# slp-rl/slamkit

Hardware: AMD Instinct MI355X
Metric: train tokens/sec (whole node), Slam-358M ctx=1024 (higher is better)
Workload: dtype bf16; 1 GPU; configs[1]: Slam-358M (Qwen2.5-0.5B body, vocab 502, rope_theta 1e4), ctx=1024, synthetic unit-token stream, random-init weights; full optimizer step (AdamW on bf16 parameters with bf16 moments); model=Slam-358M, global_batch=8, micro_batch=8, seq_len=1024, grad_accum=1, parallelism=dp1, optimizer_state_dtype=bfloat16

## Files before the change

### slamkit_amd/csrc/attention.hip

```cpp
#include <type_traits>

#include "common.h"
#include "kernels.h"

namespace {

constexpr int IMG = 64 * 128;
constexpr float NEG_BIG = -1.0e30f;
constexpr float M_INIT = -1.0e29f;
constexpr int NCH_MAX = 4;
constexpr float LN2 = 0.69314718055994530942f;

struct AttnArgs {
  const bf16_t* qkv;
  bf16_t* o;
  const bf16_t* d_o;
  bf16_t* dqkv;
  float* lse2;
  float* ndsum;
  float* nlse;
  float* dkv_part;
  const int* seg_start;
  const int* seg_end;
  const float* rope_cs;
  const float* rope_sn;
  const int* perm;
  int M, nH, nKV, ldq, nch, prio;
  float scale;
};

typedef __attribute__((address_space(3))) const char* lds_cptr_t;
typedef __attribute__((ext_vector_type(4))) unsigned u32x4_t;
typedef __attribute__((address_space(3))) const u32x4_t* lds_u4ptr_t;
SLAM_DEVICE lds_cptr_t lds_p(uint32_t a) { return (lds_cptr_t)(uintptr_t)a; }

SLAM_DEVICE int uni_f(int k) { return ((k & 3) << 1) ^ ((k >> 2) * 5); }

struct TileOff {
  uint32_t v[2];
  int ld, tid;
  SLAM_DEVICE void init(int ld_, int tid_) {
    ld = ld_; tid = tid_;
#pragma unroll
    for (int i = 0; i < 2; ++i) v[i] = off(i, 63);
  }
  SLAM_DEVICE uint32_t off(int i, int maxrow) const {
    int P = i * 256 + tid;
    int row = P >> 3, slot = P & 7;
    int c = slot ^ uni_f((row >> 1) & 7);
    row = row < maxrow ? row : maxrow;
    return (uint32_t)(((size_t)row * ld + c * 8) * sizeof(bf16_t));
  }
};
template <bool FULL>
SLAM_DEVICE void dma_tile64(const bf16_t* tb, const TileOff& to, int maxrow, uint32_t dst) {
#pragma unroll
  for (int i = 0; i < 2; ++i) glds16_m0(tb, FULL ? to.v[i] : to.off(i, maxrow), dst + (uint32_t)(i * 4096));
}

struct FragOff {
  uint32_t d[2], t[4];
  SLAM_DEVICE void init(int l15, int g) {
    const int fk = uni_f(l15 >> 1);
#pragma unroll
    for (int ds = 0; ds < 2; ++ds) d[ds] = (uint32_t)(l15 * 128 + (((g + 4 * ds) ^ fk) << 4));
    const int x = ((l15 & 3) >> 1) ^ uni_f(2 * g + (l15 >> 3));
#pragma unroll
    for (int fd = 0; fd < 4; ++fd)
      t[fd] = (uint32_t)((4 * g + (l15 >> 2)) * 128 + (((2 * fd) ^ x) << 4) + (l15 & 1) * 8);
  }
};
struct TileAddr {
  uint32_t d[2], t[4];
  SLAM_DEVICE void set(const FragOff& fo, uint32_t stage_base) {
#pragma unroll
    for (int i = 0; i < 2; ++i) { d[i] = stage_base + fo.d[i]; asm volatile("" : "+v"(d[i])); }
#pragma unroll
    for (int i = 0; i < 4; ++i) { t[i] = stage_base + fo.t[i]; asm volatile("" : "+v"(t[i])); }
  }
  SLAM_DEVICE uint4 D(int img, int f, int ds) const {
    const u32x4_t v = *(lds_u4ptr_t)(lds_p(d[ds]) + (img + f * 2048));
    return make_uint4(v[0], v[1], v[2], v[3]);
  }
  SLAM_DEVICE uint4 T(int img, int fd, int t2) const {
    lds_cptr_t q = lds_p(t[fd]) + (img + t2 * 4096);
    typedef __attribute__((address_space(3))) s16x4_t* trp_t;
    s16x4_t lo = __builtin_amdgcn_ds_read_tr16_b64_v4i16((trp_t)q);
    s16x4_t hi = __builtin_amdgcn_ds_read_tr16_b64_v4i16((trp_t)(q + 2048));
    uint2 a = __builtin_bit_cast(uint2, lo), b = __builtin_bit_cast(uint2, hi);
    return make_uint4(a.x, a.y, b.x, b.y);
  }
};

SLAM_DEVICE uint4 pack_pair(const f32x4_t& a, const f32x4_t& b) {
  return make_uint4(pack_bf16x2(a[0], a[1]), pack_bf16x2(a[2], a[3]), pack_bf16x2(b[0], b[1]),
                    pack_bf16x2(b[2], b[3]));
}
SLAM_DEVICE void wait_all_loads_visible() { __builtin_amdgcn_s_waitcnt(0x0F70); }

struct BlockItem { int slot, h, kvh; bool valid; };
SLAM_DEVICE BlockItem block_item(int b, int ntile, int nH, int nKV) {
  const int G = nH / nKV;
  const int seq = b >> 3;
  const int cid = (seq / G) * 8 + (b & 7);
  BlockItem it;
  it.valid = cid < ntile * nKV;
  it.kvh = cid % nKV;
  it.slot = cid / nKV;
  it.h = it.kvh * G + seq % G;
  return it;
}
SLAM_DEVICE void set_rank_prio(int rank, int total) {
  const int q = (4 * rank) / (total > 0 ? total : 1);
  if (q <= 0) __builtin_amdgcn_s_setprio(3);
  else if (q == 1) __builtin_amdgcn_s_setprio(2);
  else if (q == 2) __builtin_amdgcn_s_setprio(1);
}
inline int item_grid(int ntile, int nH, int nKV) { return ((ntile * nKV + 7) / 8) * 8 * (nH / nKV); }

template <int ND>
struct FwdCfg {
  static constexpr int NST = ND == 1 ? 3 : 2;
  static constexpr int STAGE = 2 * ND * IMG;
  static constexpr int OCC = ND == 1 ? 3 : 2;
};
template <int ND>
__global__ __launch_bounds__(256, FwdCfg<ND>::OCC) void attn_fwd_kernel(AttnArgs p) {
  constexpr int NST = FwdCfg<ND>::NST, STG = FwdCfg<ND>::STAGE, D = 64 * ND;
  extern __shared__ __attribute__((aligned(16))) char smem[];
  const int tid = threadIdx.x, lane = tid & 63, wave = tid >> 6;
  const int l15 = lane & 15, g = lane >> 4;
  const int M = p.M, ld = p.ldq;
// ... 148 lines not shown
    for (int j = 0; j < 2; ++j) {
      float ps = 0.f;
#pragma unroll
      for (int f = 0; f < 4; ++f)
#pragma unroll
        for (int r = 0; r < 4; ++r) {
          const float e = fast_exp2(st[f][j][r]);
          st[f][j][r] = e;
          ps += e;
        }
      lsum[j] += ps;
      pb[0][j] = pack_pair(st[0][j], st[1][j]);
      pb[1][j] = pack_pair(st[2][j], st[3][j]);
    }
    __builtin_amdgcn_sched_barrier(0);
    uint4 vf1[4 * ND];
#pragma unroll
    for (int fd = 0; fd < 4 * ND; ++fd) vf1[fd] = ta.T((ND + (fd >> 2)) * IMG, fd & 3, 1);
#pragma unroll
    for (int fd = 0; fd < 4 * ND; ++fd)
#pragma unroll
      for (int j = 0; j < 2; ++j) ot[fd][j] = mfma16(vf0[fd], pb[0][j], ot[fd][j]);
#pragma unroll
    for (int fd = 0; fd < 4 * ND; ++fd)
#pragma unroll
      for (int j = 0; j < 2; ++j) ot[fd][j] = mfma16(vf1[fd], pb[1][j], ot[fd][j]);
  }
#pragma unroll
  for (int j = 0; j < 2; ++j) {
    float l = lsum[j];
    l += __shfl_xor(l, 16, 64);
    l += __shfl_xor(l, 32, 64);
    const int q = qrow[j];
    if (q < M) {
      const float inv = 1.f / l;
#pragma unroll
      for (int fd = 0; fd < 4 * ND; ++fd) {
        uint2 o;
        o.x = pack_bf16x2(ot[fd][j][0] * inv, ot[fd][j][1] * inv);
        o.y = pack_bf16x2(ot[fd][j][2] * inv, ot[fd][j][3] * inv);
        *reinterpret_cast<uint2*>(p.o + (size_t)q * (p.nH * D) + h * D + fd * 16 + g * 4) = o;
      }
      if (g == 0 && p.lse2) p.lse2[(size_t)h * M + q] = log2f(l) - negm[j][0];
    }
  }
}

template <int ND, int JQ>
struct DqCfg {
  static constexpr int NST = ND == 1 ? 3 : 2;
  static constexpr int STAGE = 2 * ND * IMG;
  static constexpr int OCC = ND == 1 ? (JQ == 1 ? 3 : 2) : 2;
};
template <int ND, int JQ>
__global__ __launch_bounds__(256, (DqCfg<ND, JQ>::OCC)) void attn_bwd_dq_kernel(AttnArgs p) {
  constexpr int D = 64 * ND, STG = DqCfg<ND, JQ>::STAGE, NST = DqCfg<ND, JQ>::NST, QT = 64 * JQ, WR = 16 * JQ;
  extern __shared__ __attribute__((aligned(16))) char smem[];
  const int tid = threadIdx.x, lane = tid & 63, wave = tid >> 6;
  const int l15 = lane & 15, g = lane >> 4;
  const int M = p.M, ld = p.ldq;
  const BlockItem bi = block_item(blockIdx.x, (M + QT - 1) / QT, p.nH, p.nKV);
  if (!bi.valid) return;
  const int h = bi.h, kvh = bi.kvh;
  const int q0 = (p.perm ? p.perm[bi.slot] : bi.slot) * QT;
  if (p.prio && p.perm) set_rank_prio(bi.slot, (M + QT - 1) / QT);
  const int wv = __builtin_amdgcn_readfirstlane(wave);
  const int qw0 = q0 + wv * WR;
  const bf16_t* Qb = p.qkv + h * D;
  const bf16_t* Kb = p.qkv + (p.nH + kvh) * D;
  const bf16_t* Vb = p.qkv + (p.nH + p.nKV + kvh) * D;
  const float c2 = p.scale * 1.44269504088896340736f;
  const uint32_t lds0 = lds_addr(smem);

  const int kt_begin = p.seg_start[q0 < M ? q0 : M - 1] / 64;
  const int kt_end = (min(q0 + QT - 1, M - 1)) / 64;
  const int n = kt_end - kt_begin + 1;
  TileOff off;
  off.init(ld, tid);
  FragOff fo;
  fo.init(l15, g);
  const size_t tstep = (size_t)64 * ld;
  const bf16_t* kp = Kb + (size_t)kt_begin * tstep;
  const bf16_t* vp = Vb + (size_t)kt_begin * tstep;
  int irow = kt_begin * 64;
  const uint32_t wdst = lds0 + (uint32_t)wv * 1024u;
  auto issue = [&](int stage) __attribute__((always_inline)) {
    const uint32_t st = wdst + (uint32_t)(stage * STG);
    if (irow + 64 <= M) {
#pragma unroll
      for (int dh = 0; dh < ND; ++dh) {
        dma_tile64<true>(kp + dh * 64, off, 63, st + dh * IMG);
        dma_tile64<true>(vp + dh * 64, off, 63, st + (ND + dh) * IMG);
      }
    } else {
      const int mr = M - 1 - irow;
#pragma unroll
      for (int dh = 0; dh < ND; ++dh) {
        dma_tile64<false>(kp + dh * 64, off, mr, st + dh * IMG);
        dma_tile64<false>(vp + dh * 64, off, mr, st + (ND + dh) * IMG);
      }
    }
    kp += tstep; vp += tstep; irow += 64;
  };
#pragma unroll
  for (int s = 0; s < NST - 1; ++s)
    if (s < n) issue(s);

  int qrow[JQ], segs[JQ];
  float lse[JQ], nds[JQ];
  uint4 qf[JQ][2 * ND], dof[JQ][2 * ND];
#pragma unroll
  for (int j = 0; j < JQ; ++j) {
    const int q = qw0 + j * 16 + l15;
    const int qc = q < M ? q : M - 1;
    qrow[j] = q;
    segs[j] = p.seg_start[qc];
    lse[j] = -p.lse2[(size_t)h * M + qc];
    float dsm = 0.f;
#pragma unroll
    for (int ds = 0; ds < 2 * ND; ++ds) {
      qf[j][ds] = *reinterpret_cast<const uint4*>(Qb + (size_t)qc * ld + g * 8 + 32 * ds);
      dof[j][ds] = *reinterpret_cast<const uint4*>(p.d_o + (size_t)qc * p.nH * D + h * D + g * 8 + 32 * ds);
      uint4 of = *reinterpret_cast<const uint4*>(p.o + (size_t)qc * p.nH * D + h * D + g * 8 + 32 * ds);
      float x[8], y[8];
      unpack_bf16x8(dof[j][ds], x);
      unpack_bf16x8(of, y);
#pragma unroll
      for (int e = 0; e < 8; ++e) dsm += x[e] * y[e];
    }
    dsm += __shfl_xor(dsm, 16, 64);
    dsm += __shfl_xor(dsm, 32, 64);
    nds[j] = -dsm;
    if (g == 0 && q < M) {
      p.ndsum[(size_t)h * M + q] = -dsm;
      p.nlse[(size_t)h * M + q] = lse[j];
    }
  }
  const int segmax_w = p.seg_start[min(qw0 + WR - 1, M - 1)];
  f32x4_t dq[JQ][4 * ND];
#pragma unroll
  for (int j = 0; j < JQ; ++j)
#pragma unroll
    for (int fd = 0; fd < 4 * ND; ++fd) dq[j][fd] = (f32x4_t){0.f, 0.f, 0.f, 0.f};
  wait_all_loads_visible();

  int stage = 0, istage = (NST - 1) % NST;
  for (int t = 0; t < n; ++t) {
    if (NST >= 3 && t + 1 < n) wait_vmcnt<4 * ND>();
    else wait_vmcnt<0>();
    __syncthreads();
    if (t + NST - 1 < n) issue(istage);
    istage = istage + 1 == NST ? 0 : istage + 1;
    const uint32_t sb = lds0 + (uint32_t)(stage * STG);
    stage = stage + 1 == NST ? 0 : stage + 1;
    const int key0 = (kt_begin + t) * 64;
    if (key0 > qw0 + WR - 1) continue;
    TileAddr ta;
    ta.set(fo, sb);
    f32x4_t st[4][JQ], dp[4][JQ];
#pragma unroll
    for (int f = 0; f < 4; ++f)
#pragma unroll
      for (int j = 0; j < JQ; ++j) {
        st[f][j] = (f32x4_t){lse[j], lse[j], lse[j], lse[j]};
        dp[f][j] = (f32x4_t){nds[j], nds[j], nds[j], nds[j]};
      }
#pragma unroll
    for (int ds = 0; ds < 2 * ND; ++ds)
#pragma unroll
      for (int f = 0; f < 4; ++f) {
        const uint4 kf = ta.D((ds >> 1) * IMG, f, ds & 1);
        const uint4 vf = ta.D((ND + (ds >> 1)) * IMG, f, ds & 1);
#pragma unroll
        for (int j = 0; j < JQ; ++j) {
          st[f][j] = mfma16(kf, qf[j][ds], st[f][j]);
          dp[f][j] = mfma16(vf, dof[j][ds], dp[f][j]);
        }
      }
    uint4 dsb[2][JQ];
    auto soft = [&](auto mk) __attribute__((always_inline)) {
      constexpr bool MASK = decltype(mk)::value;
#pragma unroll
      for (int j = 0; j < JQ; ++j) {
        int hi = 0, lo = 0;
        if constexpr (MASK) {
          hi = (qrow[j] < M ? qrow[j] : -(1 << 30)) - key0 - 4 * g;
          lo = segs[j] - key0 - 4 * g;
        }
#pragma unroll
        for (int f = 0; f < 4; ++f)
#pragma unroll
          for (int r = 0; r < 4; ++r) {
            float pe = fast_exp2(st[f][j][r]);
            if constexpr (MASK) {
              const bool ok = (f * 16 + r <= hi) & (f * 16 + r >= lo);
              pe = ok ? pe : 0.f;
            }
            st[f][j][r] = pe * dp[f][j][r];
          }
        dsb[0][j] = pack_pair(st[0][j], st[1][j]);
        dsb[1][j] = pack_pair(st[2][j], st[3][j]);
      }
    };
    uint4 kt0[4 * ND];
#pragma unroll
    for (int fd = 0; fd < 4 * ND; ++fd) kt0[fd] = ta.T((fd >> 2) * IMG, fd & 3, 0);
    __builtin_amdgcn_sched_barrier(0);
    if ((key0 + 63 > qw0) || (key0 < segmax_w) || (qw0 + WR - 1 >= M)) soft(std::true_type{});
    else soft(std::false_type{});
    __builtin_amdgcn_sched_barrier(0);
    uint4 kt1[4 * ND];
#pragma unroll
    for (int fd = 0; fd < 4 * ND; ++fd) kt1[fd] = ta.T((fd >> 2) * IMG, fd & 3, 1);
#pragma unroll
    for (int fd = 0; fd < 4 * ND; ++fd)
#pragma unroll
      for (int j = 0; j < JQ; ++j) dq[j][fd] = mfma16(kt0[fd], dsb[0][j], dq[j][fd]);
#pragma unroll
    for (int fd = 0; fd < 4 * ND; ++fd)
#pragma unroll
      for (int j = 0; j < JQ; ++j) dq[j][fd] = mfma16(kt1[fd], dsb[1][j], dq[j][fd]);
  }
#pragma unroll
  for (int j = 0; j < JQ; ++j) {
    const int q = qrow[j];
    if (q < M) {
#pragma unroll
      for (int fd = 0; fd < 4 * ND; ++fd)
#pragma unroll
        for (int r = 0; r < 4; ++r) dq[j][fd][r] *= p.scale;
      if (p.rope_cs) {
#pragma unroll
        for (int fd = 0; fd < 2 * ND; ++fd) {
          const float4 c4 = *reinterpret_cast<const float4*>(p.rope_cs + (size_t)q * (D / 2) + fd * 16 + g * 4);
          const float4 s4 = *reinterpret_cast<const float4*>(p.rope_sn + (size_t)q * (D / 2) + fd * 16 + g * 4);
          const float cc[4] = {c4.x, c4.y, c4.z, c4.w}, ss[4] = {s4.x, s4.y, s4.z, s4.w};
#pragma unroll
          for (int r = 0; r < 4; ++r) {
            float a = dq[j][fd][r], b = dq[j][fd + 2 * ND][r];
            dq[j][fd][r] = a * cc[r] + b * ss[r];
            dq[j][fd + 2 * ND][r] = b * cc[r] - a * ss[r];
          }
        }
      }
#pragma unroll
      for (int fd = 0; fd < 4 * ND; ++fd) {
        uint2 o;
        o.x = pack_bf16x2(dq[j][fd][0], dq[j][fd][1]);
        o.y = pack_bf16x2(dq[j][fd][2], dq[j][fd][3]);
        *reinterpret_cast<uint2*>(p.dqkv + (size_t)q * ld + h * D + fd * 16 + g * 4) = o;
      }
    }
  }
}

template <int ND, int KW>
struct DkvCfg {
  static constexpr int NST = ND == 1 ? 3 : 2;
  static constexpr int STAGE = 2 * ND * IMG + 1024;
  static constexpr int OCC = ND == 1 ? (KW == 1 ? 3 : 2) : 2;
};
struct DkvRange { int qa, nq, nch; };
SLAM_DEVICE DkvRange dkv_range(const int* seg_end, int M, int k0, int KT, int nchmax, int c) {
  const int qt_begin = k0 / 64;
  const int qt_end = (seg_end[min(k0 + KT - 1, M - 1)] - 1) / 64;
  const int n = qt_end - qt_begin + 1;
  const int cs = (n + nchmax - 1) / nchmax;
  DkvRange r;
  r.nch = (n + cs - 1) / cs;
  r.qa = qt_begin + c * cs;
  r.nq = min(cs, qt_end - r.qa + 1);
  return r;
}
template <int ND, int KW>
__global__ __launch_bounds__(256, (DkvCfg<ND, KW>::OCC)) void attn_bwd_dkv_kernel(AttnArgs p) {
  constexpr int D = 64 * ND, STG = DkvCfg<ND, KW>::STAGE, NST = DkvCfg<ND, KW>::NST, KT = 64 * KW, WK = 16 * KW;
  constexpr int NDMA = 4 * ND + 1;
  extern __shared__ __attribute__((aligned(16))) char smem[];
  const int tid = threadIdx.x, lane = tid & 63, wave = tid >> 6;
  const int l15 = lane & 15, g = lane >> 4;
  const int M = p.M, ld = p.ldq, ldo = p.nH * D;
  const int G = p.nH / p.nKV;
  const int kvh = blockIdx.x % p.nKV;
  const int item = p.perm[blockIdx.x / p.nKV];
  if (item < 0) return;
  if (p.prio) set_rank_prio(blockIdx.x / p.nKV, ((M + KT - 1) / KT) * NCH_MAX);
  const int chunk = item & (NCH_MAX - 1), k0 = (item >> 2) * KT;
  const DkvRange rg = dkv_range(p.seg_end, M, k0, KT, p.nch, chunk);
  const int nq = rg.nq, qa = rg.qa;
  const int n = G * nq;
  const bf16_t* Kb = p.qkv + (p.nH + kvh) * D;
  const bf16_t* Vb = p.qkv + (p.nH + p.nKV + kvh) * D;
  const float c2 = p.scale * 1.44269504088896340736f;
  const uint32_t lds0 = lds_addr(smem);
// ... 207 lines not shown
    }
  }
  if (which == 0 && p.rope_cs) {
    const float4 c4 = *reinterpret_cast<const float4*>(p.rope_cs + (size_t)m * HALF + c * 4);
    const float4 s4 = *reinterpret_cast<const float4*>(p.rope_sn + (size_t)m * HALF + c * 4);
    float4 x = a, y = b;
    a = make_float4(x.x * c4.x + y.x * s4.x, x.y * c4.y + y.y * s4.y, x.z * c4.z + y.z * s4.z, x.w * c4.w + y.w * s4.w);
    b = make_float4(y.x * c4.x - x.x * s4.x, y.y * c4.y - x.y * s4.y, y.z * c4.z - x.z * s4.z, y.w * c4.w - x.w * s4.w);
  }
  uint2 o1, o2;
  o1.x = pack_bf16x2(a.x, a.y); o1.y = pack_bf16x2(a.z, a.w);
  o2.x = pack_bf16x2(b.x, b.y); o2.y = pack_bf16x2(b.z, b.w);
  int col = (p.nH + (which ? p.nKV : 0) + kvh) * D + c * 4;
  *reinterpret_cast<uint2*>(p.dqkv + (size_t)m * p.ldq + col) = o1;
  *reinterpret_cast<uint2*>(p.dqkv + (size_t)m * p.ldq + col + HALF) = o2;
}

__global__ __launch_bounds__(1024) void attn_plan_kernel(const int* __restrict__ seg_s, const int* __restrict__ seg_e, int M, int qt,
                                                        int kt, int nchmax, int* __restrict__ plan) {
  extern __shared__ int wk[];
  const int nf = (M + 127) / 128, nq = (M + qt - 1) / qt, nk = (M + kt - 1) / kt;
  const int total = seg_e ? nf + nq + nk * NCH_MAX : nf;
  for (int t = threadIdx.x; t < total; t += blockDim.x) {
    int w;
    if (t < nf) { int q0 = t * 128; w = min(q0 + 127, M - 1) / 64 - seg_s[q0] / 64 + 1; }
    else if (t < nf + nq) { int q0 = (t - nf) * qt; w = min(q0 + qt - 1, M - 1) / 64 - seg_s[q0] / 64 + 1; }
    else {
      const int j = t - nf - nq, c = j & (NCH_MAX - 1);
      const DkvRange r = dkv_range(seg_e, M, (j >> 2) * kt, kt, nchmax, c);
      w = c < r.nch ? r.nq : -1;
    }
    wk[t] = w;
  }
  __syncthreads();
  for (int t = threadIdx.x; t < total; t += blockDim.x) {
    int base, n;
    if (t < nf) { base = 0; n = nf; }
    else if (t < nf + nq) { base = nf; n = nq; }
    else { base = nf + nq; n = nk * NCH_MAX; }
    const int i = t - base, w = wk[t];
    int rank = 0;
    for (int j = 0; j < n; ++j) {
      const int wj = wk[base + j];
      rank += (wj > w) || (wj == w && j < i);
    }
    plan[base + rank] = (base == nf + nq && w <= 0) ? -1 : i;
  }
}

}

namespace slam {

static AttnTune g_attn_tune = {1, 1, 4, 0};
AttnTune attn_default_tune() { return g_attn_tune; }
void attn_set_default_tune(AttnTune t) { g_attn_tune = t; }
static AttnTune clamp_tune(AttnTune t, int head_dim) {
  t.jq = t.jq == 2 && head_dim == 64 ? 2 : 1;
  t.kw = 1;
  t.nch = t.nch < 1 ? 1 : t.nch > NCH_MAX ? NCH_MAX : t.nch;
  return t;
}

size_t attn_plan_ints(int M) { return (size_t)((M + 127) / 128 + (M + 63) / 64 + NCH_MAX * ((M + 63) / 64)); }
int attn_plan(const int* seg_start, const int* seg_end, int M, int head_dim, AttnTune tune, int* plan, hipStream_t st) {
  tune = clamp_tune(tune, head_dim);
  const int qt = 64 * tune.jq, kt = 64 * tune.kw;
  const int total = (M + 127) / 128 + (M + qt - 1) / qt + NCH_MAX * ((M + kt - 1) / kt);
  if ((size_t)total * sizeof(int) > 48 * 1024) return -1;
  attn_plan_kernel<<<1, 1024, (size_t)total * sizeof(int), st>>>(seg_start, seg_end, M, qt, kt, tune.nch, plan);
  return (int)hipGetLastError();
}

template <typename K>
static int set_lds(K kernel, int bytes) {
  return (int)hipFuncSetAttribute(reinterpret_cast<const void*>(kernel), hipFuncAttributeMaxDynamicSharedMemorySize, bytes);
}

template <int ND>
static int attn_fwd_nd(AttnArgs a, hipStream_t st) {
  static bool done = false;
  constexpr int lds = FwdCfg<ND>::NST * FwdCfg<ND>::STAGE;
  if (!done) { if (int e = set_lds(&attn_fwd_kernel<ND>, lds)) return e; done = true; }
  attn_fwd_kernel<ND><<<item_grid((a.M + 127) / 128, a.nH, a.nKV), 256, lds, st>>>(a);
  return (int)hipGetLastError();
}

template <int ND, int JQ>
static int attn_dq_launch(AttnArgs a, hipStream_t st) {
  static bool done = false;
  constexpr int lds = DqCfg<ND, JQ>::NST * DqCfg<ND, JQ>::STAGE;
  if (!done) { if (int e = set_lds(&attn_bwd_dq_kernel<ND, JQ>, lds)) return e; done = true; }
  attn_bwd_dq_kernel<ND, JQ><<<item_grid((a.M + 64 * JQ - 1) / (64 * JQ), a.nH, a.nKV), 256, lds, st>>>(a);
  return (int)hipGetLastError();
}
template <int ND, int KW>
static int attn_dkv_launch(AttnArgs a, hipStream_t st) {
  static bool done = false;
  constexpr int lds = DkvCfg<ND, KW>::NST * DkvCfg<ND, KW>::STAGE;
  if (!done) { if (int e = set_lds(&attn_bwd_dkv_kernel<ND, KW>, lds)) return e; done = true; }
  const int nk = (a.M + 64 * KW - 1) / (64 * KW);
  attn_bwd_dkv_kernel<ND, KW><<<nk * NCH_MAX * a.nKV, 256, lds, st>>>(a);
  return (int)hipGetLastError();
}

int attn_fwd(const bf16_t* qkv, bf16_t* o, float* lse2, const int* seg_start, const int* plan, AttnTune tune, int M, int nH,
             int nKV, int head_dim, hipStream_t st) {
  if ((head_dim != 64 && head_dim != 128) || nH % nKV) return -1;
  AttnArgs a{};
  a.qkv = qkv; a.o = o; a.lse2 = lse2; a.seg_start = seg_start; a.perm = plan; a.prio = tune.prio;
  a.M = M; a.nH = nH; a.nKV = nKV; a.ldq = (nH + 2 * nKV) * head_dim; a.scale = 1.0f / sqrtf((float)head_dim);
  return head_dim == 64 ? attn_fwd_nd<1>(a, st) : attn_fwd_nd<2>(a, st);
}

size_t attn_bwd_workspace_bytes(int M, int nKV, int head_dim) {
  return (size_t)NCH_MAX * 2 * nKV * M * head_dim * sizeof(float);
}

int attn_bwd(const bf16_t* qkv, const bf16_t* o, const bf16_t* d_o, const float* lse2, float* ndsum, float* nlse,
             bf16_t* dqkv, float* dkv_part, const int* seg_start, const int* seg_end, const int* plan, AttnTune tune,
             const float* rope_cs, const float* rope_sn, int M, int nH, int nKV, int head_dim, hipStream_t st) {
  if ((head_dim != 64 && head_dim != 128) || nH % nKV || !plan) return -1;
  tune = clamp_tune(tune, head_dim);
  AttnArgs a{};
  a.qkv = qkv; a.o = const_cast<bf16_t*>(o); a.d_o = d_o; a.dqkv = dqkv;
  a.lse2 = const_cast<float*>(lse2); a.ndsum = ndsum; a.nlse = nlse; a.dkv_part = dkv_part;
  a.seg_start = seg_start; a.seg_end = seg_end;
  a.rope_cs = rope_cs; a.rope_sn = rope_sn;
  a.M = M; a.nH = nH; a.nKV = nKV; a.ldq = (nH + 2 * nKV) * head_dim; a.scale = 1.0f / sqrtf((float)head_dim);
  a.nch = tune.nch; a.prio = tune.prio;
  const int nf = (M + 127) / 128, qt = 64 * tune.jq, kt = 64 * tune.kw;
  a.perm = plan + nf;
  int e;
  if (head_dim == 128) e = attn_dq_launch<2, 1>(a, st);
  else e = tune.jq == 2 ? attn_dq_launch<1, 2>(a, st) : attn_dq_launch<1, 1>(a, st);
  if (e) return e;
  a.perm = plan + nf + (M + qt - 1) / qt;
  if (head_dim == 128) e = attn_dkv_launch<2, 1>(a, st);
  else e = attn_dkv_launch<1, 1>(a, st);
  if (e) return e;
  const size_t total = (size_t)2 * M * nKV * (head_dim / 8);
  if (head_dim == 128) attn_dkv_reduce_kernel<2><<<(unsigned)((total + 255) / 256), 256, 0, st>>>(a, kt);
  else attn_dkv_reduce_kernel<1><<<(unsigned)((total + 255) / 256), 256, 0, st>>>(a, kt);
  return (int)hipGetLastError();
}

}
```

### slamkit_amd/csrc/engine.hip

```cpp
#include <hip/hip_runtime.h>
#include <math.h>
#include <stdio.h>
#include <dlfcn.h>
#include <string.h>

#include <algorithm>
#include <string>
#include <unordered_map>
#include <utility>
#include <vector>

#if __has_include(<rccl/rccl.h>)
#include <rccl/rccl.h>
#else
typedef struct ncclComm* ncclComm_t;
typedef struct { char internal[128]; } ncclUniqueId;
typedef enum { ncclSuccess = 0 } ncclResult_t;
typedef enum { ncclInt8 = 0, ncclUint8 = 1, ncclInt32 = 2, ncclUint32 = 3, ncclInt64 = 4, ncclUint64 = 5, ncclFloat16 = 6, ncclFloat32 = 7,
               ncclFloat64 = 8, ncclBfloat16 = 9 } ncclDataType_t;
typedef enum { ncclSum = 0 } ncclRedOp_t;
#endif

#include "../../include/slam_engine.h"
#include "kernels.h"
// ... 798 lines not shown
  if (!h->params) return h->fail(SLAM_ESTATE, "bind params first");
  hipStream_t st = (hipStream_t)stream;
  CK(join_optimizer(h, st));
  CK(join_params(h, st));
  h->params_t_dirty = false;
  const auto tr = transpose_group(h, st);
  CK(for_each_param_group(h, 0, tr));
  CK(for_each_param_group(h, h->d.n_layers + 1, tr));
  CK(for_each_layer_tensor(h, 0, h->d.n_layers, tr));
  return SLAM_OK;
}
int slam_bind_params_t(SlamEngine* h, void* params_t_bf16) {
  if (!h) return SLAM_EINVAL;
  const SlamModelDesc& d = h->d;
  if (params_t_bf16 && ((d.hidden & 63) || (d.intermediate & 63) || (h->QKV & 63) || ((d.n_heads * d.head_dim) & 63)))
    return h->fail(SLAM_EINVAL, "transposed weight images need dims that are multiples of 64");
  h->params_t = (bf16_t*)params_t_bf16;
  return SLAM_OK;
}
size_t slam_workspace_bytes(SlamEngine* h, int64_t max_tokens) {
  if (!h || max_tokens <= 0) return 0;
  GemmTuneScope tune_scope(&h->gemm_tune);
  SlamEngine tmp;
  tmp.d = h->d;
  tmp.arch = h->arch;
  tmp.npos = h->npos;
  tmp.QKV = h->QKV;
  tmp.vpad = h->vpad;
  tmp.untied = h->untied;
  tmp.n_params = h->n_params;
  tmp.recompute = h->recompute;
  tmp.dropout_thr16 = h->dropout_thr16;
  return carve(&tmp, nullptr, max_tokens);
}
int slam_bind_workspace(SlamEngine* h, void* ws, size_t bytes, int64_t max_tokens) {
  if (!h || !ws || max_tokens <= 0) return SLAM_EINVAL;
  if (((uintptr_t)ws) & 255) return h->fail(SLAM_EINVAL, "workspace must be 256-byte aligned");
  size_t need = slam_workspace_bytes(h, max_tokens);
  if (bytes < need) return h->fail(SLAM_ENOMEM, "workspace too small");
  carve(h, (char*)ws, max_tokens);
  h->ws = (char*)ws;
  h->ws_bytes = bytes;
  h->max_tokens = max_tokens;
  h->have_fwd = false;
  return SLAM_OK;
}
int slam_set_option(SlamEngine* h, const char* key, int64_t value) {
  if (!key) return SLAM_EINVAL;
  if (!strncmp(key, "gemm_", 5)) {
    const int r = gemm_tune_set(h ? &h->gemm_tune : gemm_default_tune(), key, (long)value);
    if (r > 0) return SLAM_OK;
    return h ? h->fail(SLAM_EINVAL, std::string(r < 0 ? "value out of range for option " : "unknown option ") + key) : SLAM_EINVAL;
  }
  if (!strcmp(key, "attn_jq") || !strcmp(key, "attn_kw") || !strcmp(key, "attn_nch") || !strcmp(key, "attn_prio")) {
    AttnTune t = h ? h->attn_tune : attn_default_tune();
    (key[5] == 'j' ? t.jq : key[5] == 'k' ? t.kw : key[5] == 'n' ? t.nch : t.prio) = (int)value;
    if (h) { h->attn_tune = t; h->have_fwd = false; } else attn_set_default_tune(t);
    return SLAM_OK;
  }
  if (!strcmp(key, "overlap_adamw") && h) { h->overlap_adamw = value != 0; return SLAM_OK; }
  if (!strcmp(key, "adamw_sr") && h) {
    if (value < 0 || value > 1) return h->fail(SLAM_EINVAL, "value out of range for option adamw_sr (0 or 1)");
    h->adamw_sr = (int)value;
    return SLAM_OK;
  }
  if (!strcmp(key, "adamw_sr_seed") && h) { h->adamw_sr_seed = (uint64_t)value; return SLAM_OK; }
  if (!strcmp(key, "bwd_wgrad_stream") && h) { h->wgrad_stream = value != 0; return SLAM_OK; }
  if (!strcmp(key, "bwd_aux_side") && h) { h->aux_side = value != 0; return SLAM_OK; }
  if (!strcmp(key, "bwd_wgrad_cus") && h) { h->wside_cus = (int)value; return SLAM_OK; }
  if (!strcmp(key, "time_param_waits") && h) { h->time_param_waits = value != 0; return SLAM_OK; }
  if (!strcmp(key, "time_gateup") && h) {
    if (value && h->tg_ev.empty()) {
      h->tg_ev.resize((size_t)2 * h->d.n_layers);
      for (auto& e : h->tg_ev)
        if (hipEventCreate(&e) != hipSuccess) { h->tg_ev.clear(); return h->fail(SLAM_ESTATE, "hipEventCreate failed"); }
    }
    h->time_gateup = value != 0;
    return SLAM_OK;
  }
  if (!strcmp(key, "time_families") && h) { h->time_families = value != 0; if (!value) h->fam_marks.clear(); return SLAM_OK; }
  if (!strcmp(key, "grad_overwrite_next") && h) { h->overwrite_next = value != 0; return SLAM_OK; }
  if (!strcmp(key, "grad_norm_partials") && h) { h->norm_partials = value != 0; return SLAM_OK; }
  if (!strcmp(key, "grad_final_next") && h) {
    if (value < 0 || value > 2) return h->fail(SLAM_EINVAL, "grad_final_next takes 0, 1 or 2");
    h->final_next = (int)value;
    return SLAM_OK;
  }
  if (!strcmp(key, "recompute") && h) {
    if (value < 0 || value > 2) return h->fail(SLAM_EINVAL, "value out of range for option recompute (0, 1 or 2)");
    if ((int)value != h->recompute) {
      h->recompute = (int)value;
      h->ws = nullptr;
      h->ws_bytes = 0;
      h->max_tokens = 0;
      h->have_fwd = h->have_loss = false;
      h->kv_ready = false;
    }
    return SLAM_OK;
  }
  if (!strcmp(key, "dropout_thr16") && h) {
    if (value < 0 || value > 65535) return h->fail(SLAM_EINVAL, "value out of range for option dropout_thr16 (0 .. 65535)");
    if (value != 0 && h->arch != 1) return h->fail(SLAM_EINVAL, "dropout_thr16: residual dropout exists for the OPT family only");
    if ((value != 0) != (h->dropout_thr16 != 0)) {
      h->ws = nullptr;
      h->ws_bytes = 0;
      h->max_tokens = 0;
      h->have_fwd = h->have_loss = false;
      h->kv_ready = false;
    }
// ... 1682 lines not shown
```

### slamkit_amd/csrc/kernels.h

```cpp
#pragma once
#include <hip/hip_runtime.h>
#include <stddef.h>
#include <stdint.h>

typedef uint16_t bf16_t;

namespace slam {

struct GemmTune {
  int glds = 1;
  int tn_dma = 1;
  int group_rows = 3, group_rows_256 = 4;
  int nt_store = 0;
  int g256 = 1;
  int g256_dswiglu = 1, g256_persist = 1;
  int g256_stagger = 1200, g256_stagger_dswiglu = 1200;
  int group_cols_256 = 0;
  int g256_persist_cus = 0;
  int g256_cohorts = 0;
  int shared = 0;
  int nt224 = 1, nt224_min_k = 2048;
  int tn_splits_override = 0, tn_balanced = 1, bal_bg_max_split = 4;
  int tn224 = 1, tn224_min_m = 16384, tn224_max_split = 16, tn224_bg_min_m = 4096, tn224_bg_max_split = 1;
  int mf32 = 0;
  int g256_w4 = 0;
  int g256_roles = 0;
  int g256_batch_loads = 1;
};
GemmTune* gemm_default_tune();
GemmTune* gemm_use_tune(GemmTune* t);
int gemm_tune_set(GemmTune* t, const char* key, long value);
struct GemmTuneScope {
  GemmTune* old;
  explicit GemmTuneScope(GemmTune* t) : old(gemm_use_tune(t)) {}
  ~GemmTuneScope() { gemm_use_tune(old); }
};
int gemm_nt(const bf16_t* X, const bf16_t* W, bf16_t* Y, const bf16_t* bias, const bf16_t* resid, int M, int N,
            int K, hipStream_t st);
int gemm_nt_swiglu(const bf16_t* X, const bf16_t* W, bf16_t* Y, bf16_t* act, int M, int N, int K, hipStream_t st);
int gemm_nt_rope(const bf16_t* X, const bf16_t* W, bf16_t* Y, const bf16_t* bias, const float* cs, const float* sn,
                 const float* csq, const float* snq, int q_heads, int rope_heads, int M, int N, int K, hipStream_t st);
int gemm_nt_dswiglu(const bf16_t* dY, const bf16_t* Wt, bf16_t* gu, int M, int N, int K, hipStream_t st);
int gemm_nt_relu(const bf16_t* X, const bf16_t* W, bf16_t* act, const bf16_t* bias, int M, int N, int K, hipStream_t st);
int gemm_nt_drelu(const bf16_t* dY, const bf16_t* Wt, bf16_t* dact, const bf16_t* act, int M, int N, int K, hipStream_t st);
int gemm_nn(const bf16_t* dY, const bf16_t* W, bf16_t* dX, const bf16_t* resid, int M, int N, int K,
            hipStream_t st);
int gemm_tn_splits(int M, int N, int K);
struct GradSink {
  int img_only = 0;
  float* sumsq = nullptr;
  int cap = 0;
  int used = 0;
};
size_t gemm_tn_sumsq_slots(int N, int K);
size_t gemm_tn_workspace_bytes(int M, int N, int K);
int gemm_tn(const bf16_t* dY, const bf16_t* X, float* dW, int accumulate, int M, int N, int K, int ldy, int ldx,
            float* ws, size_t ws_bytes, hipStream_t st, int background = 0, bf16_t* img = nullptr, GradSink* sink = nullptr);

struct AttnTune { int jq, kw, nch, prio; };
AttnTune attn_default_tune();
void attn_set_default_tune(AttnTune t);
size_t attn_plan_ints(int M);
int attn_plan(const int* seg_start, const int* seg_end, int M, int head_dim, AttnTune tune, int* plan, hipStream_t st);
int attn_fwd(const bf16_t* qkv, bf16_t* o, float* lse2, const int* seg_start, const int* plan, AttnTune tune, int M, int nH,
             int nKV, int head_dim, hipStream_t st);
size_t attn_bwd_workspace_bytes(int M, int nKV, int head_dim);
int attn_bwd(const bf16_t* qkv, const bf16_t* o, const bf16_t* d_o, const float* lse2, float* ndsum, float* nlse, bf16_t* dqkv,
             float* dkv_part, const int* seg_start, const int* seg_end, const int* plan, AttnTune tune,
             const float* rope_cs, const float* rope_sn, int M, int nH, int nKV, int head_dim, hipStream_t st);

int rmsnorm_fwd(const bf16_t* x, const bf16_t* w, bf16_t* y, float* rstd, int M, int H, float eps, hipStream_t st);
int layernorm_fwd(const bf16_t* x, const bf16_t* w, const bf16_t* b, bf16_t* y, float* mean, float* rstd, int M, int H, float eps,
                  hipStream_t st);
int layernorm_bwd(const bf16_t* dy, const bf16_t* x, const bf16_t* w, const float* mean, const float* rstd, const bf16_t* dres,
                  bf16_t* dx, float* dw_part, float* db_part, int M, int H, hipStream_t st);
int rmsnorm_bwd_blocks(int M);
int rmsnorm_bwd(const bf16_t* dy, const bf16_t* x, const bf16_t* w, const float* rstd, const bf16_t* dres,
                bf16_t* dx, float* dw, int accumulate, float* part, int M, int H, hipStream_t st, bf16_t* dw_img = nullptr,
                GradSink* sink = nullptr);
int colsum_blocks(int M);
int colsum_bf16(const bf16_t* X, int ld, int M, int N, float* out, int accumulate, float* part, hipStream_t st);
int rope_table(const int64_t* pos, int M, int T, int head_dim, float theta, float* cs, float* sn, float* csq, float* snq,
               float qscale, hipStream_t st);
int rope_apply(bf16_t* qkv, int ld, int M, int nrot_heads, int head_dim, const float* cs, const float* sn, int backward,
               hipStream_t st, int q_heads = 0, float q_scale = 1.f);
int qknorm_rope_fwd(bf16_t* qkv, int ld, int M, int nH, int nKV, int head_dim, const bf16_t* wq, const bf16_t* wk, const float* cs,
                    const float* sn, const float* csq, const float* snq, float eps, bf16_t* raw_save, float* rstd_save,
                    hipStream_t st);
int qknorm_bwd_blocks(int M, int nH, int nKV, int head_dim);
int qknorm_bwd(bf16_t* dqkv, int ld, int M, int nH, int nKV, int head_dim, const bf16_t* raw, const float* rstd, const bf16_t* wq,
               const bf16_t* wk, int nb, float* part_q, float* part_k, hipStream_t st);
int qknorm_rows_f32(float* qkv, int ld, int B, int nH, int nKV, int head_dim, const bf16_t* wq, const bf16_t* wk, float eps,
                    hipStream_t st);
int swiglu_fwd(const bf16_t* gu, bf16_t* act, int M, int I, int blk, hipStream_t st);
int swiglu_bwd(bf16_t* gu, const bf16_t* dact, int M, int I, int blk, hipStream_t st);
int embed_fwd(const int64_t* ids, const bf16_t* E, bf16_t* out, int M, int H, int V, hipStream_t st);
int embed_pos_fwd(const int64_t* ids, const int64_t* pos, const bf16_t* E, const bf16_t* P, bf16_t* out, int64_t* prow, int M, int H,
                  int V, int T, int NP, hipStream_t st);
int relu_bwd(bf16_t* d, const bf16_t* act, size_t n, hipStream_t st);
struct DropSite { int thr16 = 0; uint64_t seed = 0; uint32_t call = 0, site = 0; int64_t index0 = 0; };
int dropout_add(bf16_t* y, const bf16_t* resid, int M, int H, const DropSite& d, hipStream_t st);
int dropout_bwd(const bf16_t* dy, bf16_t* dm, int M, int H, const DropSite& d, hipStream_t st);
int onehot(const int64_t* ids, bf16_t* oh, int M, int Vp, int V, int pad_id, hipStream_t st);
size_t embed_bwd_workspace_ints(int M, int Vp);
int embed_bwd(const int64_t* ids, const bf16_t* dh, float* dE, int M, int H, int Vp, int V, int pad_id, int* ws,
              hipStream_t st);
int cross_entropy(const bf16_t* logits, const int64_t* labels, double num_items, bf16_t* dlogits, float* row_loss,
                  float* denom, float* loss, int B, int T, int Vp, int V, const uint8_t* colmask, float eps, float* row_smooth,
                  hipStream_t st);
int seq_loglik(const float* row_loss, const int64_t* labels, int B, int T, float* ll, float* cnt, hipStream_t st);
int copy_cols(const bf16_t* src, int lds_, bf16_t* dst, int ldd, int M, int ncols, hipStream_t st);
int scale_bf16(bf16_t* x, size_t n, float s, hipStream_t st);
// ... 190 lines not shown
```

Baseline: 339,400 tokens/s.

## Software-pipeline attention backward dQ kernel across key tiles for head_dim 64

Adds a pipelined variant of the dQ backward kernel, on by default for head_dim 64 with jq=1. It issues the next tile's K/V LDS reads and S/dP MFMAs while the current tile's softmax-gradient and dQ MFMAs run. Masking is applied before the exponent by setting masked scores to a large negative value, and the fully-masked tile skip is dropped. The aim is to hide LDS latency and the exp/pack work behind matrix ops, at the cost of more registers and a full vmcnt wait each iteration. The RoPE dQ epilogue is also rewritten with explicit FMAs.

```diff
diff --git a/slamkit_amd/csrc/attention.hip b/slamkit_amd/csrc/attention.hip
--- a/slamkit_amd/csrc/attention.hip
+++ b/slamkit_amd/csrc/attention.hip
@@ -72,12 +72,15 @@
 };
 struct TileAddr {
   uint32_t d[2], t[4];
-  SLAM_DEVICE void set(const FragOff& fo, uint32_t stage_base) {
+  SLAM_DEVICE void set_d(const FragOff& fo, uint32_t stage_base) {
 #pragma unroll
     for (int i = 0; i < 2; ++i) { d[i] = stage_base + fo.d[i]; asm volatile("" : "+v"(d[i])); }
+  }
+  SLAM_DEVICE void set_t(const FragOff& fo, uint32_t stage_base) {
 #pragma unroll
     for (int i = 0; i < 4; ++i) { t[i] = stage_base + fo.t[i]; asm volatile("" : "+v"(t[i])); }
   }
+  SLAM_DEVICE void set(const FragOff& fo, uint32_t stage_base) { set_d(fo, stage_base); set_t(fo, stage_base); }
   SLAM_DEVICE uint4 D(int img, int f, int ds) const {
     const u32x4_t v = *(lds_u4ptr_t)(lds_p(d[ds]) + (img + f * 2048));
     return make_uint4(v[0], v[1], v[2], v[3]);
@@ -332,7 +335,7 @@
   static constexpr int STAGE = 2 * ND * IMG;
   static constexpr int OCC = ND == 1 ? (JQ == 1 ? 3 : 2) : 2;
 };
-template <int ND, int JQ>
+template <int ND, int JQ, bool PIPE>
 __global__ __launch_bounds__(256, (DqCfg<ND, JQ>::OCC)) void attn_bwd_dq_kernel(AttnArgs p) {
   constexpr int D = 64 * ND, STG = DqCfg<ND, JQ>::STAGE, NST = DqCfg<ND, JQ>::NST, QT = 64 * JQ, WR = 16 * JQ;
   extern __shared__ __attribute__((aligned(16))) char smem[];
@@ -424,82 +427,178 @@
     for (int fd = 0; fd < 4 * ND; ++fd) dq[j][fd] = (f32x4_t){0.f, 0.f, 0.f, 0.f};
   wait_all_loads_visible();
 
-  int stage = 0, istage = (NST - 1) % NST;
-  for (int t = 0; t < n; ++t) {
-    if (NST >= 3 && t + 1 < n) wait_vmcnt<4 * ND>();
+  if constexpr (PIPE) {
+    static_assert(JQ == 1 && ND == 1 && NST == 3, "the pipelined loop is written for 16 rows per wave at head_dim 64");
+    f32x4_t st[4], dp[4];
+    const f32x4_t lse4 = {lse[0], lse[0], lse[0], lse[0]}, nds4 = {nds[0], nds[0], nds[0], nds[0]};
+    uint4 kfr[2][2], vfr[2][2];
+    auto rd = [&](const TileAddr& tn, int f) __attribute__((always_inline)) {
+#pragma unroll
+      for (int ds = 0; ds < 2; ++ds) {
+        kfr[f & 1][ds] = tn.D(0, f, ds);
+        vfr[f & 1][ds] = tn.D(IMG, f, ds);
+      }
+    };
+    auto mm = [&](int f) __attribute__((always_inline)) {
+      st[f] = mfma16(kfr[f & 1][0], qf[0][0], lse4);
+      dp[f] = mfma16(vfr[f & 1][0], dof[0][0], nds4);
+      st[f] = mfma16(kfr[f & 1][1], qf[0][1], st[f]);
+      dp[f] = mfma16(vfr[f & 1][1], dof[0][1], dp[f]);
+    };
+    auto premask = [&](int key0) __attribute__((always_inline)) {
+      if ((key0 + 63 > qw0) || (key0 < segmax_w) || (qw0 + WR - 1 >= M)) {
+        const int hi = (qrow[0] < M ? qrow[0] : -(1 << 30)) - key0 - 4 * g;
+        const int lo = segs[0] - key0 - 4 * g;
+#pragma unroll
+        for (int f = 0; f < 4; ++f)
+#pragma unroll
+          for (int r = 0; r < 4; ++r) {
+            const bool ok = (f * 16 + r <= hi) & (f * 16 + r >= lo);
+            st[f][r] = ok ? st[f][r] : NEG_BIG;
+          }
+      }
+    };
+    auto body = [&](auto morec, uint32_t sb, uint32_t sbn) __attribute__((always_inline)) {
+      constexpr bool MORE = decltype(morec)::value;
+      TileAddr ta, tn;
+      ta.set_t(fo, sb);
+      if constexpr (MORE) tn.set_d(fo, sbn);
+      uint4 kt0[4], kt1[4], dsb[2];
+      f32x4_t pr[4];
+#pragma unroll
+      for (int f = 0; f < 4; ++f) {
+        if constexpr (MORE) rd(tn, f);
+        if (f == 1) {
+#pragma unroll
+          for (int fd = 0; fd < 4; ++fd) kt0[fd] = ta.T(0, fd, 0);
+        }
+        if (f == 3) {
+#pragma unroll
+          for (int fd = 0; fd < 4; ++fd) kt1[fd] = ta.T(0, fd, 1);
+        }
+#pragma unroll
+        for (int r = 0; r < 4; ++r) pr[f][r] = fast_exp2(st[f][r]) * dp[f][r];
+        if (f & 1) {
+          uint4& b = dsb[f >> 1];
+          b = pack_pair(pr[f - 1], pr[f]);
+          asm volatile("" : "+v"(b.x), "+v"(b.y), "+v"(b.z), "+v"(b.w));
+        }
+        if constexpr (MORE)
+          if (f >= 1) mm(f - 1);
+        if (f >= 2) {
+#pragma unroll
+          for (int fd = 2 * f - 4; fd < 2 * f - 2; ++fd) dq[0][fd] = mfma16(kt0[fd], dsb[0], dq[0][fd]);
+        }
+        __builtin_amdgcn_sched_barrier(0);
+      }
+      if constexpr (MORE) mm(3);
+#pragma unroll
+      for (int fd = 0; fd < 4; ++fd) dq[0][fd] = mfma16(kt1[fd], dsb[1], dq[0][fd]);
+    };
+    int stage = 0, istage = NST - 1, t = 0;
+    if (n > 1) wait_vmcnt<4 * ND>();
     else wait_vmcnt<0>();
     __syncthreads();
-    if (t + NST - 1 < n) issue(istage);
-    istage = istage + 1 == NST ? 0 : istage + 1;
-    const uint32_t sb = lds0 + (uint32_t)(stage * STG);
-    stage = stage + 1 == NST ? 0 : stage + 1;
-    const int key0 = (kt_begin + t) * 64;
-    if (key0 > qw0 + WR - 1) continue;
-    TileAddr ta;
-    ta.set(fo, sb);
-    f32x4_t st[4][JQ], dp[4][JQ];
-#pragma unroll
-    for (int f = 0; f < 4; ++f)
-#pragma unroll
-      for (int j = 0; j < JQ; ++j) {
-        st[f][j] = (f32x4_t){lse[j], lse[j], lse[j], lse[j]};
-        dp[f][j] = (f32x4_t){nds[j], nds[j], nds[j], nds[j]};
-      }
-#pragma unroll
-    for (int ds = 0; ds < 2 * ND; ++ds)
+    {
+      TileAddr t0;
+      t0.set_d(fo, lds0);
 #pragma unroll
       for (int f = 0; f < 4; ++f) {
-        const uint4 kf = ta.D((ds >> 1) * IMG, f, ds & 1);
-        const uint4 vf = ta.D((ND + (ds >> 1)) * IMG, f, ds & 1);
-#pragma unroll
+        rd(t0, f);
+        mm(f);
+        __builtin_amdgcn_sched_barrier(0);
+      }
+    }
+    for (; t + 1 < n; ++t) {
+      wait_vmcnt<0>();
+      __syncthreads();
+      if (t + 2 < n) issue(istage);
+      istage = istage + 1 == NST ? 0 : istage + 1;
+      const int nstage = stage + 1 == NST ? 0 : stage + 1;
+      premask((kt_begin + t) * 64);
+      body(std::true_type{}, lds0 + (uint32_t)(stage * STG), lds0 + (uint32_t)(nstage * STG));
+      stage = nstage;
+    }
+    premask((kt_begin + t) * 64);
+    body(std::false_type{}, lds0 + (uint32_t)(stage * STG), 0u);
+  } else {
+    int stage = 0, istage = (NST - 1) % NST;
+    for (int t = 0; t < n; ++t) {
+      if (NST >= 3 && t + 1 < n) wait_vmcnt<4 * ND>();
+      else wait_vmcnt<0>();
+      __syncthreads();
+      if (t + NST - 1 < n) issue(istage);
+      istage = istage + 1 == NST ? 0 : istage + 1;
+      const uint32_t sb = lds0 + (uint32_t)(stage * STG);
+      stage = stage + 1 == NST ? 0 : stage + 1;
+      const int key0 = (kt_begin + t) * 64;
+      if (key0 > qw0 + WR - 1) continue;
+      TileAddr ta;
+      ta.set(fo, sb);
+      f32x4_t st[4][JQ], dp[4][JQ];
+  #pragma unroll
+      for (int f = 0; f < 4; ++f)
+  #pragma unroll
         for (int j = 0; j < JQ; ++j) {
-          st[f][j] = mfma16(kf, qf[j][ds], st[f][j]);
-          dp[f][j] = mfma16(vf, dof[j][ds], dp[f][j]);
-        }
-      }
-    uint4 dsb[2][JQ];
-    auto soft = [&](auto mk) __attribute__((always_inline)) {
-      constexpr bool MASK = decltype(mk)::value;
-#pragma unroll
-      for (int j = 0; j < JQ; ++j) {
-        int hi = 0, lo = 0;
-        if constexpr (MASK) {
-          hi = (qrow[j] < M ? qrow[j] : -(1 << 30)) - key0 - 4 * g;
-          lo = segs[j] - key0 - 4 * g;
-        }
-#pragma unroll
-        for (int f = 0; f < 4; ++f)
-#pragma unroll
-          for (int r = 0; r < 4; ++r) {
-            float pe = fast_exp2(st[f][j][r]);
-            if constexpr (MASK) {
-              const bool ok = (f * 16 + r <= hi) & (f * 16 + r >= lo);
-              pe = ok ? pe : 0.f;
+          st[f][j] = (f32x4_t){lse[j], lse[j], lse[j], lse[j]};
+          dp[f][j] = (f32x4_t){nds[j], nds[j], nds[j], nds[j]};
+        }
+  #pragma unroll
+      for (int ds = 0; ds < 2 * ND; ++ds)
+  #pragma unroll
+        for (int f = 0; f < 4; ++f) {
+          const uint4 kf = ta.D((ds >> 1) * IMG, f, ds & 1);
+          const uint4 vf = ta.D((ND + (ds >> 1)) * IMG, f, ds & 1);
+  #pragma unroll
+          for (int j = 0; j < JQ; ++j) {
+            st[f][j] = mfma16(kf, qf[j][ds], st[f][j]);
+            dp[f][j] = mfma16(vf, dof[j][ds], dp[f][j]);
+          }
+        }
+      uint4 dsb[2][JQ];
+      auto soft = [&](auto mk) __attribute__((always_inline)) {
+        constexpr bool MASK = decltype(mk)::value;
+  #pragma unroll
+        for (int j = 0; j < JQ; ++j) {
+          int hi = 0, lo = 0;
+          if constexpr (MASK) {
+            hi = (qrow[j] < M ? qrow[j] : -(1 << 30)) - key0 - 4 * g;
+            lo = segs[j] - key0 - 4 * g;
+          }
+  #pragma unroll
+          for (int f = 0; f < 4; ++f)
+  #pragma unroll
+            for (int r = 0; r < 4; ++r) {
+              float pe = fast_exp2(st[f][j][r]);
+              if constexpr (MASK) {
+                const bool ok = (f * 16 + r <= hi) & (f * 16 + r >= lo);
+                pe = ok ? pe : 0.f;
+              }
+              st[f][j][r] = pe * dp[f][j][r];
             }
-            st[f][j][r] = pe * dp[f][j][r];
-          }
-        dsb[0][j] = pack_pair(st[0][j], st[1][j]);
-        dsb[1][j] = pack_pair(st[2][j], st[3][j]);
-      }
-    };
-    uint4 kt0[4 * ND];
-#pragma unroll
-    for (int fd = 0; fd < 4 * ND; ++fd) kt0[fd] = ta.T((fd >> 2) * IMG, fd & 3, 0);
-    __builtin_amdgcn_sched_barrier(0);
-    if ((key0 + 63 > qw0) || (key0 < segmax_w) || (qw0 + WR - 1 >= M)) soft(std::true_type{});
-    else soft(std::false_type{});
-    __builtin_amdgcn_sched_barrier(0);
-    uint4 kt1[4 * ND];
-#pragma unroll
-    for (int fd = 0; fd < 4 * ND; ++fd) kt1[fd] = ta.T((fd >> 2) * IMG, fd & 3, 1);
-#pragma unroll
-    for (int fd = 0; fd < 4 * ND; ++fd)
-#pragma unroll
-      for (int j = 0; j < JQ; ++j) dq[j][fd] = mfma16(kt0[fd], dsb[0][j], dq[j][fd]);
-#pragma unroll
-    for (int fd = 0; fd < 4 * ND; ++fd)
-#pragma unroll
-      for (int j = 0; j < JQ; ++j) dq[j][fd] = mfma16(kt1[fd], dsb[1][j], dq[j][fd]);
+          dsb[0][j] = pack_pair(st[0][j], st[1][j]);
+          dsb[1][j] = pack_pair(st[2][j], st[3][j]);
+        }
+      };
+      uint4 kt0[4 * ND];
+  #pragma unroll
+      for (int fd = 0; fd < 4 * ND; ++fd) kt0[fd] = ta.T((fd >> 2) * IMG, fd & 3, 0);
+      __builtin_amdgcn_sched_barrier(0);
+      if ((key0 + 63 > qw0) || (key0 < segmax_w) || (qw0 + WR - 1 >= M)) soft(std::true_type{});
+      else soft(std::false_type{});
+      __builtin_amdgcn_sched_barrier(0);
+      uint4 kt1[4 * ND];
+  #pragma unroll
+      for (int fd = 0; fd < 4 * ND; ++fd) kt1[fd] = ta.T((fd >> 2) * IMG, fd & 3, 1);
+  #pragma unroll
+      for (int fd = 0; fd < 4 * ND; ++fd)
+  #pragma unroll
+        for (int j = 0; j < JQ; ++j) dq[j][fd] = mfma16(kt0[fd], dsb[0][j], dq[j][fd]);
+  #pragma unroll
+      for (int fd = 0; fd < 4 * ND; ++fd)
+  #pragma unroll
+        for (int j = 0; j < JQ; ++j) dq[j][fd] = mfma16(kt1[fd], dsb[1][j], dq[j][fd]);
+    }
   }
 #pragma unroll
   for (int j = 0; j < JQ; ++j) {
@@ -518,8 +617,16 @@
 #pragma unroll
           for (int r = 0; r < 4; ++r) {
             float a = dq[j][fd][r], b = dq[j][fd + 2 * ND][r];
-            dq[j][fd][r] = a * cc[r] + b * ss[r];
-            dq[j][fd + 2 * ND][r] = b * cc[r] - a * ss[r];
+            if constexpr (ND == 1 && JQ == 1) {
+#pragma clang fp contract(off)
+              const float as = a * ss[r], bs = b * ss[r];
+              dq[j][fd][r] = __builtin_fmaf(a, cc[r], bs);
+              if (fd == 1 && r >= 2) dq[j][fd + 2 * ND][r] = b * cc[r] - as;
+              else dq[j][fd + 2 * ND][r] = __builtin_fmaf(b, cc[r], -as);
+            } else {
+              dq[j][fd][r] = a * cc[r] + b * ss[r];
+              dq[j][fd + 2 * ND][r] = b * cc[r] - a * ss[r];
+            }
           }
         }
       }
@@ -833,13 +940,14 @@
 
 namespace slam {
 
-static AttnTune g_attn_tune = {1, 1, 4, 0};
+static AttnTune g_attn_tune = {1, 1, 4, 0, 1};
 AttnTune attn_default_tune() { return g_attn_tune; }
 void attn_set_default_tune(AttnTune t) { g_attn_tune = t; }
 static AttnTune clamp_tune(AttnTune t, int head_dim) {
   t.jq = t.jq == 2 && head_dim == 64 ? 2 : 1;
   t.kw = 1;
   t.nch = t.nch < 1 ? 1 : t.nch > NCH_MAX ? NCH_MAX : t.nch;
+  t.pipe = t.pipe && head_dim == 64 && t.jq == 1 ? 1 : 0;
   return t;
 }
 
@@ -867,12 +975,12 @@
   return (int)hipGetLastError();
 }
 
-template <int ND, int JQ>
+template <int ND, int JQ, bool PIPE = false>
 static int attn_dq_launch(AttnArgs a, hipStream_t st) {
   static bool done = false;
   constexpr int lds = DqCfg<ND, JQ>::NST * DqCfg<ND, JQ>::STAGE;
-  if (!done) { if (int e = set_lds(&attn_bwd_dq_kernel<ND, JQ>, lds)) return e; done = true; }
-  attn_bwd_dq_kernel<ND, JQ><<<item_grid((a.M + 64 * JQ - 1) / (64 * JQ), a.nH, a.nKV), 256, lds, st>>>(a);
+  if (!done) { if (int e = set_lds(&attn_bwd_dq_kernel<ND, JQ, PIPE>, lds)) return e; done = true; }
+  attn_bwd_dq_kernel<ND, JQ, PIPE><<<item_grid((a.M + 64 * JQ - 1) / (64 * JQ), a.nH, a.nKV), 256, lds, st>>>(a);
   return (int)hipGetLastError();
 }
 template <int ND, int KW>
@@ -914,7 +1022,8 @@
   a.perm = plan + nf;
   int e;
   if (head_dim == 128) e = attn_dq_launch<2, 1>(a, st);
-  else e = tune.jq == 2 ? attn_dq_launch<1, 2>(a, st) : attn_dq_launch<1, 1>(a, st);
+  else if (tune.jq == 2) e = attn_dq_launch<1, 2>(a, st);
+  else e = tune.pipe ? attn_dq_launch<1, 1, true>(a, st) : attn_dq_launch<1, 1>(a, st);
   if (e) return e;
   a.perm = plan + nf + (M + qt - 1) / qt;
   if (head_dim == 128) e = attn_dkv_launch<2, 1>(a, st);
diff --git a/slamkit_amd/csrc/engine.hip b/slamkit_amd/csrc/engine.hip
--- a/slamkit_amd/csrc/engine.hip
+++ b/slamkit_amd/csrc/engine.hip
@@ -874,9 +874,12 @@
     if (r > 0) return SLAM_OK;
     return h ? h->fail(SLAM_EINVAL, std::string(r < 0 ? "value out of range for option " : "unknown option ") + key) : SLAM_EINVAL;
   }
-  if (!strcmp(key, "attn_jq") || !strcmp(key, "attn_kw") || !strcmp(key, "attn_nch") || !strcmp(key, "attn_prio")) {
+  if (!strcmp(key, "attn_jq") || !strcmp(key, "attn_kw") || !strcmp(key, "attn_nch") || !strcmp(key, "attn_prio") ||
+      !strcmp(key, "attn_pipe")) {
     AttnTune t = h ? h->attn_tune : attn_default_tune();
-    (key[5] == 'j' ? t.jq : key[5] == 'k' ? t.kw : key[5] == 'n' ? t.nch : t.prio) = (int)value;
+    if (!strcmp(key, "attn_pipe") && (value < 0 || value > 1))
+      return h ? h->fail(SLAM_EINVAL, "value out of range for option attn_pipe (0 or 1)") : SLAM_EINVAL;
+    (key[5] == 'j' ? t.jq : key[5] == 'k' ? t.kw : key[5] == 'n' ? t.nch : key[6] == 'i' ? t.pipe : t.prio) = (int)value;
     if (h) { h->attn_tune = t; h->have_fwd = false; } else attn_set_default_tune(t);
     return SLAM_OK;
   }
diff --git a/slamkit_amd/csrc/kernels.h b/slamkit_amd/csrc/kernels.h
--- a/slamkit_amd/csrc/kernels.h
+++ b/slamkit_amd/csrc/kernels.h
@@ -57,7 +57,7 @@
 int gemm_tn(const bf16_t* dY, const bf16_t* X, float* dW, int accumulate, int M, int N, int K, int ldy, int ldx,
             float* ws, size_t ws_bytes, hipStream_t st, int background = 0, bf16_t* img = nullptr, GradSink* sink = nullptr);
 
-struct AttnTune { int jq, kw, nch, prio; };
+struct AttnTune { int jq, kw, nch, prio, pipe; };
 AttnTune attn_default_tune();
 void attn_set_default_tune(AttnTune t);
 size_t attn_plan_ints(int M);
```

Result: no change. 339,600 tokens/s, median of 2 (+0.1%).
